# SEU-dynamical-models/Manifold-based-optical-flow-method

Measured on AMD Instinct MI355X. Metric: flow timesteps/sec on 160k-vertex mesh, higher is better.
Workload: dtype f32

## Files before the change

include/mof.h:

```cpp
#ifndef MOF_H_
#define MOF_H_

#include <stdint.h>

#ifdef __cplusplus
extern "C" {
#endif

#define MOF_ABI_VERSION 4

#define MOF_OK 0
#define MOF_E_ARG (-1)
#define MOF_E_HIP (-2)
#define MOF_E_NOCONV (-3)
#define MOF_E_STATE (-4)

#define MOF_GEOM_F32_POINTS 1u
#define MOF_NO_REORDER 2u

#define MOF_PREC_F64 0
#define MOF_PREC_MIXED 1

#define MOF_IO_DEVICE 1u
#define MOF_NO_BLOCK_JACOBI 2u
// ... 114 lines not shown

int mof_csv_write(const char *path, const double *data, int64_t rows, int64_t cols,
                  int32_t threads);
int mof_csv_shape(const char *path, int64_t *rows, int64_t *cols);
#define MOF_CSV_ROUND_TRIP 1u
int mof_csv_read(const char *path, double *out, int64_t rows, int64_t cols, uint32_t flags,
                 int32_t threads);

int mof_ply_info(const char *path, int64_t *n_vertices, int64_t *n_faces, uint32_t *has_normals);
int mof_ply_read(const char *path, float *points, int64_t *triangles, float *normals);
int mof_point_normals(const float *points, const int64_t *triangles, int64_t N, int64_t M,
                      float *normals);
int mof_cell_areas(const float *points, const int64_t *triangles, int64_t N, int64_t M,
                   double *areas);

int mof_amg_probe(const int32_t *tri, const double *e, int32_t N, int32_t M, int32_t *n_levels,
                  int32_t *level_nodes, double *qtq_err, double *max_curl);

int mof_index_probe(const int32_t *tri, int32_t N, int32_t M, uint32_t flags, int32_t sym, int64_t *sell_nb,
                    int32_t *sell_off, int32_t *col, int32_t *mir, uint32_t *packed, int32_t *sym_used,
                    int32_t *packed_used);
int mof_test_force_index32(int32_t on);

int mof_xcd_map_check(int32_t nblk, int32_t batch, int32_t group);
int mof_xcd_batch_cap(int64_t nblk, int32_t group, int32_t *batch);

typedef struct mof_dd mof_dd;

typedef struct mof_dd_info {
    int32_t nparts;
    int32_t local_parts;
    int32_t rank;
    int32_t max_neighbours;
    int32_t max_owned;
    int32_t pad_;
    int64_t ghost_rows;
    int64_t send_rows;
    double ms_setup;
} mof_dd_info;

#define MOF_DD_ID_BYTES 128

int mof_partition_rcb(const double *xyz, int32_t N, int32_t nparts, int32_t *part);

int mof_dd_plan_info(const int32_t *tri, int32_t N, int32_t M, int32_t nparts, const int32_t *part,
                     int32_t *n_own, int32_t *n_ghost, int32_t *n_nbr, int32_t *n_tri,
// ... 37 lines not shown
```

manifold-based-optical-flow-method_amd/csrc/mof_abi.cpp:

```cpp
#include <algorithm>
#include <chrono>
#include <cmath>
#include <cstring>
#include <cstdio>
#include <cstdlib>
#include <functional>
#include <future>
#include <memory>
#include <mutex>
#include <new>

#include "mof_amg.h"
#include "mof_dd.h"
#include "mof_hostio.h"
#include "mof_internal.h"

namespace {

thread_local std::string g_err;

template <class F>
int guarded(F &&f) {
    try {
        f();
// ... 324 lines not shown
                release_f64();
                break;
            }
            used_f64 = true;
        } else {
            ensure(prec);
        }
        st.iterations += solve(rp, only.data());
        for (int32_t b = 0; b < nb; ++b)
            if (only[b] && !failed(b) && prec == MOF_PREC_F64) st.recovered_f64++;
    }
    if (used_f64) release_f64();
    for (int32_t b = 0; b < nb; ++b)
        if (first[b] && !failed(b)) st.recovered++;
}

}

int mof_io_guard(const std::function<void()> &f) { return guarded(f); }

namespace mof {

std::atomic<int> g_force_index32{0};

void mesh_set_own(mof_mesh *m, int32_t nown) {
    MOF_HIP(hipSetDevice(m->device));
    m->n_own = nown;
    const int sym = knob(Knob::SymReads) ? (knob_int(Knob::SymReads, 0) != 0) : -1;
    std::shared_ptr<const MirrorTable> mt;
    {
        MeshShared *sh = m->shared.get();
        std::unique_lock<std::mutex> lk;
        if (sh) lk = std::unique_lock<std::mutex>(sh->mu);
        if (sh && sh->mirror && sh->mirror->nown == nown && sh->mirror->sym == sym) {
            mt = sh->mirror;
        } else {
            auto t = std::make_shared<MirrorTable>();
            t->nown = nown;
            t->sym = sym;
            t->table = sell_mirror(m->pat, nown, sym, &t->used);
            if (t->used) t->packed = sell_index_pack(m->pat, t->table);
            if (sh) sh->mirror = t;
            mt = t;
        }
    }
    m->sym_reads = mt->used;
    const std::vector<int32_t> &mir = mt->table;
    m->sell_mir.alloc(mir.size());
    m->sell_mir.upload(mir.data(), mir.size(), m->stream);
    m->idx_packed = !mt->packed.empty() && !g_force_index32.load();
    if (m->idx_packed) {
        m->sell_idx.alloc(mt->packed.size());
        m->sell_idx.upload(mt->packed.data(), mt->packed.size(), m->stream);
    }
    int64_t own = 0;
    for (int32_t v : mir) own += v >= 0 && !(v & kMirT);
    m->blocks_read = own;
    MOF_HIP(hipStreamSynchronize(m->stream));
}

constexpr int32_t kRowsPerWindow = 256;

void mesh_prepare_host(mof_mesh *m, const double *xyz, const double *nrm, const int32_t *tri,
                       const double *area, int32_t N, int32_t M, uint32_t flags, const int32_t *perm_in,
                       const int32_t *tri_ids) {
    m->N = N;
    m->n_own = N;
    m->M = M;
    m->flags = flags;
    double t0 = now_ms();
    MOF_REQUIRE(N > 0 && M > 0, "mesh needs N > 0 vertices and M > 0 triangles");
    for (int64_t q = 0; q < 3 * (int64_t)M; ++q)
        MOF_REQUIRE(tri[q] >= 0 && tri[q] < N, "triangle vertex index out of range");
    m->perm.resize(N);
    m->tperm.resize(M);
    for (int32_t i = 0; i < N; ++i) m->perm[i] = i;
    for (int32_t T = 0; T < M; ++T) m->tperm[T] = T;
// ... 692 lines not shown
        const std::vector<double> zero(3 * (size_t)std::max(N, M), 0.0);
        mof::mesh_prepare_host(&m, zero.data(), zero.data(), tri, zero.data(), N, M, flags, nullptr, nullptr);
        const mof::Pattern &P = m.pat;
        bool used = false;
        const std::vector<int32_t> table = mof::sell_mirror(P, N, sym < 0 ? -1 : (sym != 0), &used);
        const std::vector<uint32_t> pk = used ? mof::sell_index_pack(P, table) : std::vector<uint32_t>();
        *sell_nb = P.sell_nb();
        if (sym_used) *sym_used = used;
        if (packed_used) *packed_used = !pk.empty();
        if (sell_off) std::copy(P.sell_off.begin(), P.sell_off.end(), sell_off);
        if (col) std::copy(P.sell_col.begin(), P.sell_col.end(), col);
        if (mir) std::copy(table.begin(), table.end(), mir);
        if (packed) {
            std::fill(packed, packed + P.sell_nb(), 0u);
            std::copy(pk.begin(), pk.end(), packed);
        }
    });
}

int mof_test_force_index32(int32_t on) {
    return guarded([&] { mof::g_force_index32.store(on != 0); });
}

int mof_xcd_map_check(int32_t nblk, int32_t batch, int32_t group) {
    return guarded([&] {
        MOF_REQUIRE(nblk > 0 && batch > 0 && group >= 0, "bad arguments");
        MOF_REQUIRE(mof::xcd_map_covers(nblk, batch, group), "XCD order does not cover every (row block, system) once");
    });
}

int mof_xcd_batch_cap(int64_t nblk, int32_t group, int32_t *batch) {
    return guarded([&] {
        MOF_REQUIRE(nblk > 0 && group >= 0 && batch, "bad arguments");
        *batch = mof::xcd_batch_cap_host(nblk, group);
    });
}

int mof_bench_spmv(mof_mesh *m, uint32_t precision, int32_t batch, int32_t reps,
                   double *ms_per_launch, double *bytes_per_launch) {
    return guarded([&] {
        MOF_REQUIRE(m && ms_per_launch && bytes_per_launch, "NULL argument");
        MOF_REQUIRE(reps > 0, "reps must be positive");
        mof::mesh_join_prep(m);
        DeviceGuard dg(m->device);
        *ms_per_launch = mof::bench_spmv(m, precision, batch, reps, m->stream, bytes_per_launch);
    });
// ... 4 lines not shown
```

manifold-based-optical-flow-method_amd/csrc/mof_internal.h:

```cpp
#pragma once

#include <hip/hip_runtime.h>

#include <atomic>
#include <cstdint>
#include <cstdlib>
#include <functional>
#include <future>
#include <memory>
#include <mutex>
#include <string>
#include <type_traits>
#include <vector>

#include "../../include/mof.h"
#include "mof_knobs.h"

namespace mof {

constexpr int kWG = 256;
constexpr int kSlice = 64;

struct Error {
    int code;
// ... 54 lines not shown
    std::vector<int32_t> vptr, vcol;
    std::vector<int32_t> cptr, clist;
    int32_t nslices = 0;
    std::vector<int32_t> sell_off;
    std::vector<int32_t> sell_col;
    std::vector<int32_t> sell_blk;
    std::vector<int32_t> blk_row;
    std::vector<int32_t> diag_pos;
    std::vector<int32_t> tsell_off;
    std::vector<int32_t> tinc;
    std::vector<int32_t> tslot;
    int32_t max_w = 0;
    int64_t sell_nb() const { return sell_off.empty() ? 0 : sell_off.back(); }
    int64_t tsell_nb() const { return tsell_off.empty() ? 0 : tsell_off.back(); }
    int32_t nblocks() const { return (int32_t)vcol.size(); }
};

void build_pattern(const int32_t *tri, int32_t N, int32_t M, Pattern &pat,
                   const int32_t *torder = nullptr);
std::vector<int32_t> rcm_order(const Pattern &pat);
std::vector<int32_t> sell_mirror(const Pattern &pat, int32_t nown, int sym, bool *used);
std::vector<uint32_t> sell_index_pack(const Pattern &pat, const std::vector<int32_t> &mir);
extern std::atomic<int> g_force_index32;

struct Workspace {
    int32_t cap = 0;
    int32_t nblk = 0;
    DevArray<double> u64, fc;
    DevArray<float> u32;
    DevArray<float> A32;
    DevArray<double> A64;
    DevArray<double> dinv64;
    DevArray<float> dinv32;
    DevArray<double> rhs;
    DevArray<double> x64, r64;
    DevArray<double> vx, vr, vz, vp, vq;
    DevArray<double> part_pq;
    DevArray<double> part_rzrr;
    DevArray<double> part_rr0;
    DevArray<double> part_dx;
    DevArray<double> sc;
    DevArray<double> sysd;
    DevArray<int32_t> sysi;
    DevArray<int32_t> smap;
    DevArray<double> dt;
    DevArray<double> Ibuf;
    DevArray<double> Iint;
    DevArray<double> Vbuf;
    bool u64_stale = false;
    const double *J0 = nullptr, *J1 = nullptr;
    int32_t JB = 0;
};


enum SysD { SD_TOL2 = 0, SD_RR = 1, SD_FF = 2, SD_REL = 3, SD_RR0 = 4, SD_BEST = 5, SD_OUTER = 6, SD_EST = 7,
            SD_XMAX = 8 };
enum SysI { SI_CONV = 0, SI_ACTIVE = 1, SI_FAILED = 2, SI_ITSUM = 3, SI_BEST_IT = 4, SI_FAIL_IT = 5, SI_FAIL_WHY = 6,
            SI_ITMAX = 7, SI_MET = 8 };
enum FailWhy { FW_BREAKDOWN = 1, FW_DIVERGED = 2, FW_STALLED = 3, FW_MAXITER = 4, FW_RESIDUAL = 5 };
constexpr int kSysStride = 12;

struct AmgDevice;
// ... 26 lines not shown

struct mof_mesh {
    int32_t N = 0, M = 0, device = 0;
    std::mutex prep_mu;
    std::future<void> prep;
    std::exception_ptr prep_err;
    int32_t n_own = 0;
    uint32_t flags = 0;
    hipStream_t stream = nullptr;
    mof::Pattern pat;
    std::vector<int32_t> perm, inv;
    std::vector<int32_t> tperm, tinv;
    std::vector<int32_t> agg_order;
    mof::DevArray<int32_t> perm_d;
    mof::DevArray<int32_t> tri_orig;
    mof::DevArray<int32_t> icol;
    mof::DevArray<int32_t> tri, vptr, vcol, cptr, clist, sell_off, sell_col, sell_blk, blk_row,
        diag_pos, tsell_off, tinc, tslot;
    mof::DevArray<int32_t> sell_mir;
    int64_t blocks_read = 0;
    bool sym_reads = false;
    mof::DevArray<uint32_t> sell_idx;
    bool idx_packed = false;
    mof::DevArray<double> e, gw, iw, area, a2;
    mof::DevArray<double> a2s64, w12_64;
    mof::DevArray<float> a2s32, w12_32;
    double a2s_lambda = 0.0;
    bool a2s_valid = false;
    mof::DevArray<double> Aexp, fexp;
    mof::Workspace ws;
    bool have_last_A = false;
    double ms_geometry = 0.0, ms_pattern = 0.0;
    int32_t *h_sysi = nullptr;
    double *h_sysd = nullptr;
    int32_t h_cap = 0;
    std::vector<hipEvent_t> spmv_events;
    std::vector<int32_t> iter_hint;
    mof::AmgDevice *amg = nullptr;
    mof::HostStage *stage = nullptr;
    mof::DevArray<double> hin[2], hout[2];
    std::shared_ptr<mof::MeshShared> shared;
    hipEvent_t hev[6] = {nullptr, nullptr, nullptr, nullptr, nullptr, nullptr};
    mof::WaveState *wave = nullptr;
    mof::StreamState *sline = nullptr;
};

// ... 105 lines not shown
```

manifold-based-optical-flow-method_amd/csrc/mof_pattern.cpp:

```cpp
#include <algorithm>
#include <chrono>

#include "mof_internal.h"

namespace mof {

void build_pattern(const int32_t *tri, int32_t N, int32_t M, Pattern &pat, const int32_t *torder) {
    MOF_REQUIRE(N > 0 && M > 0, "mesh needs N > 0 vertices and M > 0 triangles");
    MOF_REQUIRE((int64_t)M * 9 < (int64_t)INT32_MAX, "too many triangles for int32 term codes");
    for (int64_t q = 0; q < 3 * (int64_t)M; ++q)
        MOF_REQUIRE(tri[q] >= 0 && tri[q] < N, "triangle vertex index out of range");
    pat.N = N;
    pat.M = M;

    std::vector<int64_t> inc(N + 1, 0);
    for (int64_t q = 0; q < 3 * (int64_t)M; ++q) inc[tri[q] + 1]++;
    for (int32_t i = 0; i < N; ++i) inc[i + 1] += inc[i];
    std::vector<int32_t> cand(3 * inc[N] + N);
    std::vector<int64_t> cfill(N);
    std::vector<int64_t> cbase(N + 1);
    for (int32_t i = 0; i <= N; ++i) cbase[i] = 3 * inc[i] + i;
    for (int32_t i = 0; i < N; ++i) {
        cfill[i] = cbase[i];
        cand[cfill[i]++] = i;
// ... 179 lines not shown
}

std::vector<uint32_t> sell_index_pack(const Pattern &pat, const std::vector<int32_t> &mir) {
    const int64_t snb = pat.sell_off[pat.nslices];
    if (snb >= kIdxMaxNb || (int64_t)mir.size() != snb) return {};
    std::vector<uint32_t> out((size_t)snb, (uint32_t)(uint16_t)kIdxPad << 16);
    for (int32_t s = 0; s < pat.nslices; ++s) {
        const int32_t w = (pat.sell_off[s + 1] - pat.sell_off[s]) / kSlice;
        for (int32_t l = 0; l < kSlice; ++l) {
            const int32_t i = s * kSlice + l;
            if (i >= pat.N) break;
            for (int32_t t = 0; t < w; ++t) {
                const int64_t pos = pat.sell_off[s] + (int64_t)t * kSlice + l;
                if (mir[pos] < 0) continue;
                const int64_t dcol = (int64_t)pat.sell_col[pos] - i;
                const int64_t dpos = (int64_t)(mir[pos] & kMirPos) - pos;
                const bool tr = (mir[pos] & kMirT) != 0;
                if (dcol < -32768 || dcol > 32767 || dpos <= kIdxPad || dpos > 32767 || tr != (dpos != 0)) return {};
                out[pos] = (uint32_t)(uint16_t)(int16_t)dcol | ((uint32_t)(uint16_t)(int16_t)dpos << 16);
            }
        }
    }
    return out;
}

std::vector<int32_t> rcm_order(const Pattern &pat) {
    const int32_t N = pat.N;
    std::vector<int32_t> deg(N), order, perm(N, -1);
    order.reserve(N);
    for (int32_t i = 0; i < N; ++i) deg[i] = pat.vptr[i + 1] - pat.vptr[i];
    std::vector<int32_t> level(N, -1), queue;
    queue.reserve(N);
    auto far = [&](int32_t s) {
        std::vector<int32_t> seen_list{s};
        level[s] = 0;
        size_t h = 0;
        int32_t last = s;
        while (h < seen_list.size()) {
            const int32_t v = seen_list[h++];
            if (level[v] > level[last] || (level[v] == level[last] && deg[v] < deg[last])) last = v;
            for (int32_t q = pat.vptr[v]; q < pat.vptr[v + 1]; ++q) {
                const int32_t w = pat.vcol[q];
                if (level[w] < 0) {
                    level[w] = level[v] + 1;
                    seen_list.push_back(w);
                }
// ... 34 lines not shown
```

manifold-based-optical-flow-method_amd/csrc/mof_pcg.hip:

```cpp
#include <algorithm>
#include <cstdio>
#include <cstdlib>
#include <chrono>
#include <cmath>

#include <hip/hip_ext.h>

#include "mof_dd.h"
#include "mof_internal.h"
#include "mof_rowkern.h"

namespace mof {

thread_local double g_fetch_ms = 0.0;
thread_local int64_t g_fetch_n = 0;

namespace {

template <typename V>
struct OpArgs {
    int32_t N, M;
    const int32_t *sell_off, *sell_col;
    const V *a2s;
    const int32_t *tsell_off;
// ... 114 lines not shown
#pragma unroll
            for (int u = 0; u < U; ++u) {
                const int c = q[u].y;
                const V2 ui = c == 0 ? P0[u] : (c == 1 ? P1[u] : P2[u]);
                const V2 uj = c == 0 ? P1[u] : (c == 1 ? P2[u] : P0[u]);
                const V2 uk = c == 0 ? P2[u] : (c == 1 ? P0[u] : P1[u]);
                const V si = ui.x * xi.x + ui.y * xi.y;
                const V sj = uj.x * xj[u].x + uj.y * xj[u].y;
                const V sk = uk.x * xk[u].x + uk.y * xk[u].y;
                const V cc = (t0 + u < w) ? w12[u] * ((si + si) + sj + sk) : (V)0;
                a0 += ui.x * cc;
                a1 += ui.y * cc;
            }
        }
    }
    y0 = a0;
    y1 = a1;
}

__device__ __forceinline__ double dot3_np(const double *x, const double *y) {
    return fma(x[2], y[2], fma(x[1], y[1], __dmul_rn(x[0], y[0])));
}

template <int NS>
__device__ __forceinline__ void rcn_a2(const OpArgs<double> &op, const int32_t (&bs)[NS], int32_t i,
                                       const double *__restrict__ x64, double (&acc)[NS][2]) {
#pragma clang fp contract(off)
    const int32_t s = i >> 6, l = i & 63;
    const int32_t o = op.sell_off[s];
    const int32_t w = (op.sell_off[s + 1] - o) >> 6;
    for (int32_t t0 = 0; t0 < w; t0 += kResU) {
        int32_t j[kResU];
        double blk[kResU][4];
#pragma unroll
        for (int u = 0; u < kResU; ++u) j[u] = op.sell_col[(int64_t)o + min(t0 + u, w - 1) * kSlice + l];
#pragma unroll
        for (int u = 0; u < kResU; ++u) ld_blk(op.a2s, (int64_t)o + min(t0 + u, w - 1) * kSlice + l, blk[u]);
#pragma unroll
        for (int u = 0; u < kResU; ++u) {
            const bool on = t0 + u < w;
#pragma unroll
            for (int t = 0; t < NS; ++t) {
                const double2 xj = ld2(x64 + 2 * ((int64_t)bs[t] * op.N + j[u]));
                acc[t][0] += on ? blk[u][0] * xj.x + blk[u][1] * xj.y : 0.0;
                acc[t][1] += on ? blk[u][2] * xj.x + blk[u][3] * xj.y : 0.0;
            }
        }
    }
}
template <int NS>
struct RcnRow {
    double2 xi[NS];
    double Ii[NS];
    double ei[6];
};
template <int NS>
__device__ __forceinline__ void rcn_row(const OpArgs<double> &op, const int32_t (&bs)[NS], int32_t i,
                                        const double *__restrict__ x64, RcnRow<NS> &R) {
#pragma unroll
    for (int t = 0; t < NS; ++t) {
        R.xi[t] = ld2(x64 + 2 * ((int64_t)bs[t] * op.N + i));
        R.Ii[t] = op.I0[(int64_t)bs[t] * op.ldI + i];
    }
#pragma unroll
    for (int q = 0; q < 6; ++q) R.ei[q] = op.e[6 * (int64_t)i + q];
}
template <int NS>
__device__ __forceinline__ void rcn_tri(const OpArgs<double> &op, const int32_t (&bs)[NS], int4 q,
                                        const double *__restrict__ x64, const RcnRow<NS> &R,
                                        double (&val)[NS][2]) {
#pragma clang fp contract(off)
    double g[9], ej[6], ek[6], Ij[NS], Ik[NS], wt;
    double2 xj[NS], xk[NS];
    const int64_t T = min(q.x, op.M - 1);
#pragma unroll
    for (int k = 0; k < 9; ++k) g[k] = op.gw[9 * T + k];
#pragma unroll
    for (int k = 0; k < 6; ++k) {
        ej[k] = op.e[6 * (int64_t)q.z + k];
        ek[k] = op.e[6 * (int64_t)q.w + k];
    }
#pragma unroll
    for (int t = 0; t < NS; ++t) {
        const double *Ib = op.I0 + (int64_t)bs[t] * op.ldI;
        const int64_t vb = (int64_t)bs[t] * op.N;
        Ij[t] = Ib[q.z];
        Ik[t] = Ib[q.w];
        xj[t] = ld2(x64 + 2 * (vb + q.z));
        xk[t] = ld2(x64 + 2 * (vb + q.w));
    }
    wt = op.w12[q.x];
    const int c = q.y;
#pragma unroll
    for (int t = 0; t < NS; ++t) {
        const double c0 = c == 0 ? R.Ii[t] : (c == 1 ? Ik[t] : Ij[t]);
        const double c1 = c == 0 ? Ij[t] : (c == 1 ? R.Ii[t] : Ik[t]);
        const double c2 = c == 0 ? Ik[t] : (c == 1 ? Ij[t] : R.Ii[t]);
        double gI[3];
#pragma unroll
        for (int d = 0; d < 3; ++d) gI[d] = (c0 * g[d] + c1 * g[3 + d]) + c2 * g[6 + d];
        const double2 ui = make_double2(dot3_np(gI, R.ei), dot3_np(gI, R.ei + 3));
        const double2 uj = make_double2(dot3_np(gI, ej), dot3_np(gI, ej + 3));
        const double2 uk = make_double2(dot3_np(gI, ek), dot3_np(gI, ek + 3));
        const double si = ui.x * R.xi[t].x + ui.y * R.xi[t].y;
        const double sj = uj.x * xj[t].x + uj.y * xj[t].y;
        const double sk = uk.x * xk[t].x + uk.y * xk[t].y;
        const double cc = wt * ((si + si) + sj + sk);
        val[t][0] = ui.x * cc;
        val[t][1] = ui.y * cc;
    }
}

template <int NS>
__device__ __forceinline__ void apply_row_rcn(const OpArgs<double> &op, const int32_t (&bs)[NS], int32_t i,
                                              const double *__restrict__ x64, double (&y)[NS][2]) {
#pragma clang fp contract(off)
    static_assert(kRcU == 1, "one incidence per load batch");
    const int32_t s = i >> 6, l = i & 63;
    double acc[NS][2];
#pragma unroll
    for (int t = 0; t < NS; ++t) acc[t][0] = acc[t][1] = 0.0;
    rcn_a2<NS>(op, bs, i, x64, acc);
    RcnRow<NS> R;
    rcn_row<NS>(op, bs, i, x64, R);
    const int32_t o = op.tsell_off[s];
    const int32_t w = (op.tsell_off[s + 1] - o) >> 6;
    if (kRcPre && w <= kRcPre) {
        constexpr int P = kRcPre > 0 ? kRcPre : 1;
        int4 qs[P];
#pragma unroll
        for (int t0 = 0; t0 < P; ++t0)
            if (t0 < w) qs[t0] = op.tinc[(int64_t)o + t0 * kSlice + l];
#pragma unroll
// ... 480 lines not shown
            ff += f.x * f.x + f.y * f.y;
        }
    }
    double v[2] = {rr, ff};
    block_sum_q<2, NQ>(v, lds);
    if (tid == 0 && rb < rd.nmax) {
        double *o = part + 2 * red_rec(rd, B, b, rb);
        o[0] = v[0];
        o[1] = v[1];
    }
}
__global__ __launch_bounds__(kWG) void k_residual(OpArgs<double> op, int32_t nblk, int32_t B, RedArgs rd,
                                                  const double *__restrict__ rhs,
                                                  const double *__restrict__ x64,
                                                  const int32_t *__restrict__ sysi,
                                                  double *__restrict__ r64,
                                                  double *__restrict__ part) {
    int32_t rb, b;
    if (!xcd_map(nblk, B, rb, b, kGrpRes)) return;
    residual_rows<1>(op, B, rd, rhs, x64, sysi, r64, part, rb, b);
}

constexpr int kResNS = 2;
template <int NS>
__global__ __launch_bounds__(kWG) void k_residual_rcn(OpArgs<double> op, int32_t nblk, int32_t B, RedArgs rd,
                                                      const double *__restrict__ rhs,
                                                      const double *__restrict__ x64,
                                                      const int32_t *__restrict__ sysi,
                                                      double *__restrict__ r64,
                                                      double *__restrict__ part) {
    __shared__ double lds[8 * NS];
    int32_t rb, bp;
    if (!xcd_map(nblk, (B + NS - 1) / NS, rb, bp, kGrpRes)) return;
    int32_t bs[NS];
    bool act[NS], any = false;
#pragma unroll
    for (int t = 0; t < NS; ++t) {
        bs[t] = min(NS * bp + t, B - 1);
        act[t] = NS * bp + t < B && sysi[bs[t] * kSysStride + SI_ACTIVE] != 0;
        any |= act[t];
    }
    if (!any) return;
    const int32_t N = op.N;
    double v[2 * NS];
#pragma unroll
    for (int t = 0; t < 2 * NS; ++t) v[t] = 0.0;
#pragma unroll
    for (int r = 0; r < kRows; ++r) {
        const int32_t i = rb * kRowsPerWG + r * kWG + threadIdx.x;
        if (i >= N) break;
        double y[NS][2];
        apply_row_rcn<NS>(op, bs, i, x64, y);
#pragma unroll
        for (int t = 0; t < NS; ++t) {
            const int64_t vi = (int64_t)bs[t] * N + i;
            const double2 f = *reinterpret_cast<const double2 *>(rhs + 2 * vi);
            const double r0 = f.x - y[t][0], r1 = f.y - y[t][1];
            if (act[t]) *reinterpret_cast<double2 *>(r64 + 2 * vi) = make_double2(r0, r1);
            if (i < rd.nown) {
                v[2 * t] += r0 * r0 + r1 * r1;
                v[2 * t + 1] += f.x * f.x + f.y * f.y;
            }
        }
    }
    block_sum<2 * NS>(v, lds);
    if (threadIdx.x == 0) {
#pragma unroll
        for (int t = 0; t < NS; ++t) {
            if (!act[t]) continue;
            double *o = part + 2 * red_rec(rd, B, bs[t], rb);
            o[0] = v[2 * t];
            o[1] = v[2 * t + 1];
        }
    }
}

template <int NT = kWG>
__device__ __forceinline__ void reduce_max_sys(const double *part, const RedArgs &rdx, int32_t B, int32_t b,
                                               double (&out)[2], double *lds) {
    out[0] = out[1] = 0.0;
    for (int32_t q = 0; q < rdx.P; ++q) {
        const double *p = part + 2 * ((int64_t)q * B + b) * rdx.nmax;
        for (int32_t w = threadIdx.x; w < rdx.nmax; w += NT) {
            out[0] = fmax(out[0], p[2 * (int64_t)w]);
            out[1] = fmax(out[1], p[2 * (int64_t)w + 1]);
        }
    }
    block_max<2, NT>(out, lds);
}

template <int NT = kWG>
__device__ __forceinline__ void outer_check_sys(const RedArgs &rd, int32_t B, const double *__restrict__ part,
                                                const RedArgs &rdx, const double *__restrict__ part_dx,
                                                int32_t first, double rtol, double etol,
                                                double *__restrict__ sysd, int32_t *__restrict__ sysi,
                                                int32_t b) {
    __shared__ double lds[2 * (NT / 64)];
// ... 88 lines not shown
    op.e = m->e.p;
    op.I0 = m->ws.J0;
    op.ldI = m->N;
    return op;
}

OpArgs<double> op64(mof_mesh *m) {
    return make_op<double>(m, m->a2s64.p, m->w12_64.p, m->ws.u64_stale ? nullptr : m->ws.u64.p);
}

template <typename V>
MatArgs<V> make_mat(mof_mesh *m, const V *A) {
    MatArgs<V> mt;
    mt.sell_nb = m->pat.sell_nb();
    mt.sell_off = m->sell_off.p;
    mt.sell_col = m->sell_col.p;
    mt.sell_mir = m->sym_reads ? m->sell_mir.p : nullptr;
    mt.sell_idx = sizeof(V) == 4 && m->sym_reads && m->idx_packed ? m->sell_idx.p : nullptr;
    mt.vptr = m->sym_reads ? nullptr : m->vptr.p;
    mt.A = A;
    return mt;
}

template <typename... Args>
void launch_residual(mof_mesh *m, int32_t nblk, int32_t B, hipStream_t s, RedArgs rd, Args... args) {
    const OpArgs<double> op = op64(m);
    if (op.u)
        k_residual<<<dim3(xcd_grid(nblk, B, kGrpRes)), kWG, 0, s>>>(op, nblk, B, rd, args...);
    else
        k_residual_rcn<kResNS><<<dim3(xcd_grid(nblk, (B + kResNS - 1) / kResNS, kGrpRes)), kWG, 0, s>>>(
            op, nblk, B, rd, args...);
}

template <typename V>
PcgArgs<V> make_args(mof_mesh *m, int32_t B, const MatArgs<V> &mat, const V *dinv) {
    Workspace &w = m->ws;
    PcgArgs<V> a;
    a.N = m->N;
    a.nblk = w.nblk;
    a.B = B;
    a.sm = sys_all(B);
    a.selfred = 0;
    a.mat = mat;
    a.dinv = dinv;
    a.x = reinterpret_cast<V *>(w.vx.p);
    a.r = reinterpret_cast<V *>(w.vr.p);
    a.z = reinterpret_cast<V *>(w.vz.p);
    a.p = reinterpret_cast<V *>(w.vp.p);
    a.q = reinterpret_cast<V *>(w.vq.p);
    a.part_pq = w.part_pq.p;
    a.part_rzrr = w.part_rzrr.p;
    a.sysd = w.sysd.p;
    a.sysi = w.sysi.p;
    a.red = RedArgs{1, 0, w.nblk, m->N};
// ... 341 lines not shown
        MOF_HIP(hipStreamSynchronize(m->stream));
        return;
    }
    w.cap = B;
    w.nblk = (int32_t)((N + kRowsPerWG - 1) / kRowsPerWG);
    w.u64.release();
    w.u32.release();
    w.fc.release();
    w.dinv64.alloc(4 * N * B);
    w.dinv32.alloc(4 * N * B);
    w.rhs.alloc(2 * N * B);
    w.x64.alloc(2 * N * B);
    w.r64.alloc(2 * N * B);
    w.vx.alloc(2 * N * B);
    w.vr.alloc(2 * N * B);
    w.vz.alloc(2 * N * B);
    w.vp.alloc(2 * N * B);
    w.vq.alloc(2 * N * B);
    w.part_pq.alloc(2 * (size_t)w.nblk * B);
    w.part_rzrr.alloc((size_t)4 * w.nblk * B);
    w.sc.alloc((size_t)6 * B);
    w.sc.zero(m->stream);
    w.part_rr0.alloc((size_t)2 * w.nblk * B);
    w.part_dx.alloc((size_t)2 * ((N + kWG - 1) / kWG) * B);
    w.sysd.alloc((size_t)kSysStride * B);
    w.sysi.alloc((size_t)kSysStride * B);
    w.smap.alloc((size_t)B);
    w.dt.alloc(B);
    w.Ibuf.alloc(2 * N * B);
    w.Iint.alloc(2 * N * B);
    w.Vbuf.alloc(2 * N * B);
    if (m->h_cap < B) {
        if (m->h_sysi) (void)hipHostFree(m->h_sysi);
        if (m->h_sysd) (void)hipHostFree(m->h_sysd);
        m->h_sysi = nullptr;
        m->h_sysd = nullptr;
        MOF_HIP(hipHostMalloc((void **)&m->h_sysi, sizeof(int32_t) * kSysStride * B, 0));
        MOF_HIP(hipHostMalloc((void **)&m->h_sysd, sizeof(double) * kSysStride * B, 0));
        m->h_cap = B;
    }
    MOF_HIP(hipStreamSynchronize(m->stream));
}

constexpr int32_t kFusedMaxBlk = 16;
bool fused_eligible(const mof_mesh *m, const SolveParams &sp, const uint8_t *only) {
    if (sp.fused == 0 || only || sp.precision != MOF_PREC_F64 || sp.amg || sp.fail_at_max_iter) return false;
// ... 417 lines not shown
```

manifold-based-optical-flow-method_amd/mofhip/_lib.py:

```python
from __future__ import annotations

import ctypes
import os
import subprocess
import threading

import numpy as np

PKG_DIR = os.path.dirname(os.path.abspath(__file__))
ROOT_DIR = os.path.dirname(PKG_DIR)
CSRC_DIR = os.path.join(ROOT_DIR, "csrc")
LIB_PATH = os.environ.get("MOFHIP_LIB") or os.path.join(PKG_DIR, "libmofhip.so")

MOF_ABI_VERSION = 4

MOF_OK = 0
MOF_E_ARG = -1
MOF_E_HIP = -2
MOF_E_NOCONV = -3
MOF_E_STATE = -4

MOF_GEOM_F32_POINTS = 1
MOF_NO_REORDER = 2
MOF_PREC_F64 = 0
# ... 3 lines not shown
MOF_TIME_SPMV = 4
MOF_PRECOND_AMG = 8
MOF_NO_RECOVERY = 16
MOF_SOLVE_FUSED = 128
MOF_SOLVE_EAGER = 256
MOF_CSV_ROUND_TRIP = 1
MOF_COORDS_F32 = 32
MOF_DD_STAGED = 64
MOF_WAVE_PHASE = 512
MOF_CSR_A2 = 0
MOF_CSR_A_LAST = 1

EXPORTS = (
    "mof_version", "mof_abi_version", "mof_last_error", "mof_device_count", "mof_mesh_create", "mof_mesh_clone",
    "mof_mesh_destroy", "mof_mesh_get_info", "mof_geometry_export", "mof_csr_export",
    "mof_assemble", "mof_solve_range", "mof_bench_spmv", "mof_velocity_vectors",
    "mof_csv_write", "mof_csv_shape", "mof_csv_read", "mof_ply_info", "mof_ply_read",
    "mof_point_normals", "mof_cell_areas", "mof_singularities", "mof_amg_probe",
    "mof_partition_rcb", "mof_dd_plan_info", "mof_dd_create", "mof_dd_unique_id",
    "mof_dd_create_rank", "mof_dd_destroy", "mof_dd_get_info", "mof_dd_solve_range",
    "mof_dd_test_fail_recovery_alloc", "mof_mesh_prepare", "mof_mesh_sync",
    "mof_singularities_compact", "mof_xcd_map_check", "mof_xcd_batch_cap", "mof_dd_create_rank_host",
    "mof_index_probe", "mof_test_force_index32", "mof_wave_speed", "mof_streamline_map", "mof_streamlines",
    "mof_test_streamline_pass",
)


class MofError(RuntimeError):

    def __init__(self, code, msg):
        super().__init__("libmofhip error %d: %s" % (code, msg))
        self.code = code


class NotConverged(MofError):
    pass


class MofOpts(ctypes.Structure):
    _fields_ = [
        ("struct_size", ctypes.c_uint32), ("precision", ctypes.c_uint32),
        ("flags", ctypes.c_uint32), ("batch", ctypes.c_int32), ("max_iter", ctypes.c_int32),
        ("max_outer", ctypes.c_int32), ("rtol", ctypes.c_double),
        ("inner_rtol", ctypes.c_double), ("stream", ctypes.c_void_p),
        ("etol", ctypes.c_double),
    ]

# ... 83 lines not shown
            "mof_mesh_get_info": ([P, P], ctypes.c_int),
            "mof_geometry_export": ([P, P, P, P], ctypes.c_int),
            "mof_csr_export": ([P, i32, i32, P, P, P, P], ctypes.c_int),
            "mof_assemble": ([P, P, P, f64, f64, P], ctypes.c_int),
            "mof_solve_range": ([P, P, P, P, i32, i32, i32, f64, P, P, P], ctypes.c_int),
            "mof_bench_spmv": ([P, u32, i32, i32, P, P], ctypes.c_int),
            "mof_velocity_vectors": ([i32, P, P, i32, i32, P, P, u32, P], ctypes.c_int),
            "mof_csv_write": ([ctypes.c_char_p, P, i64, i64, i32], ctypes.c_int),
            "mof_csv_shape": ([ctypes.c_char_p, P, P], ctypes.c_int),
            "mof_csv_read": ([ctypes.c_char_p, P, i64, i64, u32, i32], ctypes.c_int),
            "mof_ply_info": ([ctypes.c_char_p, P, P, P], ctypes.c_int),
            "mof_ply_read": ([ctypes.c_char_p, P, P, P], ctypes.c_int),
            "mof_point_normals": ([P, P, i64, i64, P], ctypes.c_int),
            "mof_cell_areas": ([P, P, i64, i64, P], ctypes.c_int),
            "mof_wave_speed": ([P, P, i32, f64, u32, i32, P, P, P, P, P], ctypes.c_int),
            "mof_streamline_map": ([P, P, i32, u32, P, P, P], ctypes.c_int),
            "mof_streamlines": ([P, P, i32, i32, u32, P, i64, i64, P, P, P, P], ctypes.c_int),
            "mof_test_streamline_pass": ([i32], ctypes.c_int),
            "mof_singularities": ([i32, P, P, i32, i32, P, i32, f64, u32, P, P, P, P, P],
                                  ctypes.c_int),
            "mof_amg_probe": ([P, P, i32, i32, P, P, P, P], ctypes.c_int),
            "mof_index_probe": ([P, i32, i32, u32, i32, P, P, P, P, P, P, P], ctypes.c_int),
            "mof_test_force_index32": ([i32], ctypes.c_int),
            "mof_xcd_map_check": ([i32, i32, i32], ctypes.c_int),
            "mof_xcd_batch_cap": ([i64, i32, P], ctypes.c_int),
            "mof_singularities_compact": ([i32, P, P, i32, i32, P, i32, f64, u32, P, i64, P, P, P, P, P,
                                           P, P], ctypes.c_int),
            "mof_partition_rcb": ([P, i32, i32, P], ctypes.c_int),
            "mof_dd_plan_info": ([P, i32, i32, i32, P, P, P, P, P, P], ctypes.c_int),
            "mof_dd_create": ([P, P, P, P, i32, i32, i32, P, i32, u32, P], ctypes.c_int),
            "mof_dd_unique_id": ([P], ctypes.c_int),
            "mof_dd_create_rank": ([P, P, P, P, i32, i32, i32, P, i32, P, i32, u32, P],
                                   ctypes.c_int),
            "mof_dd_create_rank_host": ([P, P, P, P, i32, i32, i32, P, i32, P, i32, u32, P],
                                        ctypes.c_int),
            "mof_dd_destroy": ([P], ctypes.c_int),
            "mof_dd_get_info": ([P, P], ctypes.c_int),
            "mof_mesh_prepare": ([P, P], ctypes.c_int),
            "mof_mesh_sync": ([P], ctypes.c_int),
            "mof_dd_test_fail_recovery_alloc": ([P, i32], ctypes.c_int),
            "mof_dd_solve_range": ([P, P, P, P, i32, i32, i32, f64, P, P, P], ctypes.c_int),
        }
        for name, (args, res) in sig.items():
            if os.environ.get("MOFHIP_LIB") and not hasattr(L, name):
                continue
            fn = getattr(L, name)
# ... 33 lines not shown
```

manifold-based-optical-flow-method_amd/mofhip/mesh.py:

```python
from __future__ import annotations

import ctypes
import threading
import time

import numpy as np

from . import _lib as L


def _f64(a):
    return np.ascontiguousarray(a, dtype=np.float64)


class DeviceMesh:

    def __init__(self, coordinates, normals, triangles, areas, device: int = 0,
                 reorder: bool = True):
        coords = np.asarray(coordinates)
        tri = np.asarray(triangles)
        if coords.ndim != 2 or coords.shape[1] != 3:
            raise ValueError("coordinates must be (N, 3)")
        if tri.ndim != 2 or tri.shape[1] != 3:
            raise ValueError("triangles must be (M, 3)")
# ... 234 lines not shown
    flags = 0 if reorder else L.MOF_NO_REORDER
    nb, su, pu = ctypes.c_int64(0), ctypes.c_int32(0), ctypes.c_int32(0)
    L.check(L.lib().mof_index_probe(L.ptr(T), N, M, flags, int(sym), ctypes.byref(nb), None, None, None, None,
                                    None, None))
    off = np.zeros((N + 63) // 64 + 1, dtype=np.int32)
    col = np.zeros(nb.value, dtype=np.int32)
    mir = np.zeros(nb.value, dtype=np.int32)
    packed = np.zeros(nb.value, dtype=np.uint32)
    L.check(L.lib().mof_index_probe(L.ptr(T), N, M, flags, int(sym), ctypes.byref(nb), L.ptr(off), L.ptr(col),
                                    L.ptr(mir), L.ptr(packed), ctypes.byref(su), ctypes.byref(pu)))
    return {"sell_off": off, "col": col, "mir": mir, "packed": packed, "sym_used": bool(su.value),
            "packed_used": bool(pu.value)}


class force_index32:

    def __enter__(self):
        L.check(L.lib().mof_test_force_index32(1))
        return self

    def __exit__(self, *exc):
        L.check(L.lib().mof_test_force_index32(0))
        return False
```

Before: 4033.

## Stage per-slice operator data in LDS for batched residual kernel

Adds a residual kernel that loads one 64-row slice's A2 blocks, column indices, edge frames and triangle incidence/gradient data into shared memory once. Several waves then reuse that staged data across multiple system pairs, and a small fold kernel reduces the per-slice partial norms into the existing reduction records. The aim is to cut repeated global reads of matrix and geometry data across systems in the batch. The cost is a large dynamic LDS allocation per block (up to 160 KB), which limits occupancy, plus an extra launch and workspace buffer. The older per-row kernel remains as a fallback when a slice does not fit.

```diff
diff --git a/include/mof.h b/include/mof.h
--- a/include/mof.h
+++ b/include/mof.h
@@ -160,6 +160,12 @@
                     int32_t *packed_used);
 int mof_test_force_index32(int32_t on);
 
+int mof_residual_probe(const int32_t *tri, int32_t N, int32_t M, uint32_t flags, int64_t *staged_bytes,
+                       int32_t *staged_used);
+int mof_test_force_residual_rows(int32_t on);
+int mof_test_force_residual_trips(int32_t on);
+int mof_test_residual_launches(int64_t *counts);
+
 int mof_xcd_map_check(int32_t nblk, int32_t batch, int32_t group);
 int mof_xcd_batch_cap(int64_t nblk, int32_t group, int32_t *batch);
 
diff --git a/manifold-based-optical-flow-method_amd/csrc/mof_abi.cpp b/manifold-based-optical-flow-method_amd/csrc/mof_abi.cpp
--- a/manifold-based-optical-flow-method_amd/csrc/mof_abi.cpp
+++ b/manifold-based-optical-flow-method_amd/csrc/mof_abi.cpp
@@ -370,6 +370,9 @@
 namespace mof {
 
 std::atomic<int> g_force_index32{0};
+std::atomic<int> g_force_residual_rows{0};
+std::atomic<int> g_force_residual_trips{0};
+std::atomic<int64_t> g_residual_launches[3];
 
 void mesh_set_own(mof_mesh *m, int32_t nown) {
     MOF_HIP(hipSetDevice(m->device));
@@ -401,6 +404,8 @@
         m->sell_idx.alloc(mt->packed.size());
         m->sell_idx.upload(mt->packed.data(), mt->packed.size(), m->stream);
     }
+    m->res_lds_bytes = res_staged_bytes(m->pat);
+    m->res_lds = m->res_lds_bytes <= kResLdsCap && !g_force_residual_rows.load();
     int64_t own = 0;
     for (int32_t v : mir) own += v >= 0 && !(v & kMirT);
     m->blocks_read = own;
@@ -1139,6 +1144,33 @@
     return guarded([&] { mof::g_force_index32.store(on != 0); });
 }
 
+int mof_residual_probe(const int32_t *tri, int32_t N, int32_t M, uint32_t flags, int64_t *staged_bytes,
+                       int32_t *staged_used) {
+    return guarded([&] {
+        MOF_REQUIRE(tri && staged_bytes && N > 0 && M > 0, "bad arguments");
+        mof_mesh m;
+        const std::vector<double> zero(3 * (size_t)std::max(N, M), 0.0);
+        mof::mesh_prepare_host(&m, zero.data(), zero.data(), tri, zero.data(), N, M, flags, nullptr, nullptr);
+        *staged_bytes = mof::res_staged_bytes(m.pat);
+        if (staged_used) *staged_used = *staged_bytes <= mof::kResLdsCap;
+    });
+}
+
+int mof_test_force_residual_rows(int32_t on) {
+    return guarded([&] { mof::g_force_residual_rows.store(on != 0); });
+}
+
+int mof_test_force_residual_trips(int32_t on) {
+    return guarded([&] { mof::g_force_residual_trips.store(on != 0); });
+}
+
+int mof_test_residual_launches(int64_t *counts) {
+    return guarded([&] {
+        MOF_REQUIRE(counts, "NULL argument");
+        for (int k = 0; k < 3; ++k) counts[k] = mof::g_residual_launches[k].load();
+    });
+}
+
 int mof_xcd_map_check(int32_t nblk, int32_t batch, int32_t group) {
     return guarded([&] {
         MOF_REQUIRE(nblk > 0 && batch > 0 && group >= 0, "bad arguments");
diff --git a/manifold-based-optical-flow-method_amd/csrc/mof_internal.h b/manifold-based-optical-flow-method_amd/csrc/mof_internal.h
--- a/manifold-based-optical-flow-method_amd/csrc/mof_internal.h
+++ b/manifold-based-optical-flow-method_amd/csrc/mof_internal.h
@@ -100,6 +100,14 @@
 std::vector<int32_t> sell_mirror(const Pattern &pat, int32_t nown, int sym, bool *used);
 std::vector<uint32_t> sell_index_pack(const Pattern &pat, const std::vector<int32_t> &mir);
 extern std::atomic<int> g_force_index32;
+constexpr int64_t kResLdsCap = 160 * 1024;
+inline int64_t res_slice_bytes(int32_t w_a2, int32_t w_inc) {
+    return (int64_t)kSlice * ((int64_t)w_a2 * 36 + (int64_t)w_inc * 192 + 48);
+}
+int64_t res_staged_bytes(const Pattern &pat);
+extern std::atomic<int> g_force_residual_rows;
+extern std::atomic<int> g_force_residual_trips;
+extern std::atomic<int64_t> g_residual_launches[3];
 
 struct Workspace {
     int32_t cap = 0;
@@ -116,6 +124,7 @@
     DevArray<double> part_pq;
     DevArray<double> part_rzrr;
     DevArray<double> part_rr0;
+    DevArray<double> res_spart;
     DevArray<double> part_dx;
     DevArray<double> sc;
     DevArray<double> sysd;
@@ -188,6 +197,8 @@
     bool sym_reads = false;
     mof::DevArray<uint32_t> sell_idx;
     bool idx_packed = false;
+    int64_t res_lds_bytes = 0;
+    bool res_lds = false;
     mof::DevArray<double> e, gw, iw, area, a2;
     mof::DevArray<double> a2s64, w12_64;
     mof::DevArray<float> a2s32, w12_32;
diff --git a/manifold-based-optical-flow-method_amd/csrc/mof_pattern.cpp b/manifold-based-optical-flow-method_amd/csrc/mof_pattern.cpp
--- a/manifold-based-optical-flow-method_amd/csrc/mof_pattern.cpp
+++ b/manifold-based-optical-flow-method_amd/csrc/mof_pattern.cpp
@@ -225,6 +225,14 @@
         }
     }
     return out;
+}
+
+int64_t res_staged_bytes(const Pattern &pat) {
+    int64_t mx = 0;
+    for (int32_t s = 0; s < pat.nslices; ++s)
+        mx = std::max(mx, res_slice_bytes((pat.sell_off[s + 1] - pat.sell_off[s]) / kSlice,
+                                          (pat.tsell_off[s + 1] - pat.tsell_off[s]) / kSlice));
+    return mx;
 }
 
 std::vector<int32_t> rcm_order(const Pattern &pat) {
diff --git a/manifold-based-optical-flow-method_amd/csrc/mof_pcg.hip b/manifold-based-optical-flow-method_amd/csrc/mof_pcg.hip
--- a/manifold-based-optical-flow-method_amd/csrc/mof_pcg.hip
+++ b/manifold-based-optical-flow-method_amd/csrc/mof_pcg.hip
@@ -160,6 +160,11 @@
     return fma(x[2], y[2], fma(x[1], y[1], __dmul_rn(x[0], y[0])));
 }
 
+__device__ __forceinline__ void rcn_a2_term(const double (&blk)[4], double2 xj, bool on, double (&acc)[2]) {
+#pragma clang fp contract(off)
+    acc[0] += on ? blk[0] * xj.x + blk[1] * xj.y : 0.0;
+    acc[1] += on ? blk[2] * xj.x + blk[3] * xj.y : 0.0;
+}
 template <int NS>
 __device__ __forceinline__ void rcn_a2(const OpArgs<double> &op, const int32_t (&bs)[NS], int32_t i,
                                        const double *__restrict__ x64, double (&acc)[NS][2]) {
@@ -178,11 +183,8 @@
         for (int u = 0; u < kResU; ++u) {
             const bool on = t0 + u < w;
 #pragma unroll
-            for (int t = 0; t < NS; ++t) {
-                const double2 xj = ld2(x64 + 2 * ((int64_t)bs[t] * op.N + j[u]));
-                acc[t][0] += on ? blk[u][0] * xj.x + blk[u][1] * xj.y : 0.0;
-                acc[t][1] += on ? blk[u][2] * xj.x + blk[u][3] * xj.y : 0.0;
-            }
+            for (int t = 0; t < NS; ++t)
+                rcn_a2_term(blk[u], ld2(x64 + 2 * ((int64_t)bs[t] * op.N + j[u])), on, acc[t]);
         }
     }
 }
@@ -203,6 +205,27 @@
 #pragma unroll
     for (int q = 0; q < 6; ++q) R.ei[q] = op.e[6 * (int64_t)i + q];
 }
+__device__ __forceinline__ void rcn_tri_term(int c, const double (&g)[9], const double (&ei)[6],
+                                             const double (&ej)[6], const double (&ek)[6], double wt, double Ii,
+                                             double Ij, double Ik, double2 xi, double2 xj, double2 xk,
+                                             double (&val)[2]) {
+#pragma clang fp contract(off)
+    const double c0 = c == 0 ? Ii : (c == 1 ? Ik : Ij);
+    const double c1 = c == 0 ? Ij : (c == 1 ? Ii : Ik);
+    const double c2 = c == 0 ? Ik : (c == 1 ? Ij : Ii);
+    double gI[3];
+#pragma unroll
+    for (int d = 0; d < 3; ++d) gI[d] = (c0 * g[d] + c1 * g[3 + d]) + c2 * g[6 + d];
+    const double2 ui = make_double2(dot3_np(gI, ei), dot3_np(gI, ei + 3));
+    const double2 uj = make_double2(dot3_np(gI, ej), dot3_np(gI, ej + 3));
+    const double2 uk = make_double2(dot3_np(gI, ek), dot3_np(gI, ek + 3));
+    const double si = ui.x * xi.x + ui.y * xi.y;
+    const double sj = uj.x * xj.x + uj.y * xj.y;
+    const double sk = uk.x * xk.x + uk.y * xk.y;
+    const double cc = wt * ((si + si) + sj + sk);
+    val[0] = ui.x * cc;
+    val[1] = ui.y * cc;
+}
 template <int NS>
 __device__ __forceinline__ void rcn_tri(const OpArgs<double> &op, const int32_t (&bs)[NS], int4 q,
                                         const double *__restrict__ x64, const RcnRow<NS> &R,
@@ -228,25 +251,8 @@
         xk[t] = ld2(x64 + 2 * (vb + q.w));
     }
     wt = op.w12[q.x];
-    const int c = q.y;
-#pragma unroll
-    for (int t = 0; t < NS; ++t) {
-        const double c0 = c == 0 ? R.Ii[t] : (c == 1 ? Ik[t] : Ij[t]);
-        const double c1 = c == 0 ? Ij[t] : (c == 1 ? R.Ii[t] : Ik[t]);
-        const double c2 = c == 0 ? Ik[t] : (c == 1 ? Ij[t] : R.Ii[t]);
-        double gI[3];
-#pragma unroll
-        for (int d = 0; d < 3; ++d) gI[d] = (c0 * g[d] + c1 * g[3 + d]) + c2 * g[6 + d];
-        const double2 ui = make_double2(dot3_np(gI, R.ei), dot3_np(gI, R.ei + 3));
-        const double2 uj = make_double2(dot3_np(gI, ej), dot3_np(gI, ej + 3));
-        const double2 uk = make_double2(dot3_np(gI, ek), dot3_np(gI, ek + 3));
-        const double si = ui.x * R.xi[t].x + ui.y * R.xi[t].y;
-        const double sj = uj.x * xj[t].x + uj.y * xj[t].y;
-        const double sk = uk.x * xk[t].x + uk.y * xk[t].y;
-        const double cc = wt * ((si + si) + sj + sk);
-        val[t][0] = ui.x * cc;
-        val[t][1] = ui.y * cc;
-    }
+#pragma unroll
+    for (int t = 0; t < NS; ++t) rcn_tri_term(q.y, g, R.ei, ej, ek, wt, R.Ii[t], Ij[t], Ik[t], R.xi[t], xj[t], xk[t], val[t]);
 }
 
 template <int NS>
@@ -773,6 +779,17 @@
 }
 
 constexpr int kResNS = 2;
+__device__ __forceinline__ void rcn_out(int64_t vi, bool own, bool act, const double (&y)[2],
+                                        const double *__restrict__ rhs, double *__restrict__ r64, double &rr,
+                                        double &ff) {
+    const double2 f = *reinterpret_cast<const double2 *>(rhs + 2 * vi);
+    const double r0 = f.x - y[0], r1 = f.y - y[1];
+    if (act) *reinterpret_cast<double2 *>(r64 + 2 * vi) = make_double2(r0, r1);
+    if (own) {
+        rr += r0 * r0 + r1 * r1;
+        ff += f.x * f.x + f.y * f.y;
+    }
+}
 template <int NS>
 __global__ __launch_bounds__(kWG) void k_residual_rcn(OpArgs<double> op, int32_t nblk, int32_t B, RedArgs rd,
                                                       const double *__restrict__ rhs,
@@ -804,14 +821,7 @@
         apply_row_rcn<NS>(op, bs, i, x64, y);
 #pragma unroll
         for (int t = 0; t < NS; ++t) {
-            const int64_t vi = (int64_t)bs[t] * N + i;
-            const double2 f = *reinterpret_cast<const double2 *>(rhs + 2 * vi);
-            const double r0 = f.x - y[t][0], r1 = f.y - y[t][1];
-            if (act[t]) *reinterpret_cast<double2 *>(r64 + 2 * vi) = make_double2(r0, r1);
-            if (i < rd.nown) {
-                v[2 * t] += r0 * r0 + r1 * r1;
-                v[2 * t + 1] += f.x * f.x + f.y * f.y;
-            }
+            rcn_out((int64_t)bs[t] * N + i, i < rd.nown, act[t], y[t], rhs, r64, v[2 * t], v[2 * t + 1]);
         }
     }
     block_sum<2 * NS>(v, lds);
@@ -824,6 +834,183 @@
             o[1] = v[2 * t + 1];
         }
     }
+}
+
+constexpr int kLdsW = 16, kLdsTrips = 4;
+constexpr int kLdsUA = 4;
+constexpr int32_t kGrpResLds = 1;
+constexpr int64_t kLdsFill = 1024;
+template <int NS, int W, int TRIPS>
+__global__ __launch_bounds__(64 * W) void k_residual_lds(OpArgs<double> op, int32_t nsl, int32_t B, RedArgs rd,
+                                                         const double *__restrict__ rhs,
+                                                         const double *__restrict__ x64,
+                                                         const int32_t *__restrict__ sysi,
+                                                         double *__restrict__ r64,
+                                                         double *__restrict__ spart) {
+    extern __shared__ double2 sm[];
+    constexpr int NT = 64 * W, PW = W * TRIPS;
+    const int32_t npair = (B + NS - 1) / NS;
+    int32_t s, chunk;
+    if (!xcd_map(nsl, (npair + PW - 1) / PW, s, chunk, kGrpResLds)) return;
+    const int32_t wv = threadIdx.x >> 6, l = threadIdx.x & 63;
+    {
+        bool any = false;
+        for (int32_t q = l; q < PW * NS; q += 64) {
+            const int32_t b = chunk * PW * NS + q;
+            any |= b < B && sysi[min(b, B - 1) * kSysStride + SI_ACTIVE] != 0;
+        }
+        if (__ballot(any) == 0) return;
+    }
+    const int32_t N = op.N;
+    const int32_t o = op.sell_off[s], wa = (op.sell_off[s + 1] - o) >> 6;
+    const int32_t to = op.tsell_off[s], wt = (op.tsell_off[s + 1] - to) >> 6;
+    double2 *const E = sm, *const BLK = sm + 3 * 64, *const INC = BLK + 2 * 64 * wa;
+    int32_t *const COL = reinterpret_cast<int32_t *>(INC + 12 * 64 * wt);
+    for (int32_t q = threadIdx.x; q < wa * 64; q += NT) {
+        const int32_t t = q >> 6, ll = q & 63;
+        COL[q] = op.sell_col[(int64_t)o + q];
+        const double2 *bp = reinterpret_cast<const double2 *>(op.a2s) + 2 * ((int64_t)o + q);
+        BLK[(2 * t) * 64 + ll] = bp[0];
+        BLK[(2 * t + 1) * 64 + ll] = bp[1];
+    }
+    for (int32_t q = threadIdx.x; q < 3 * 64; q += NT) {
+        const int32_t k = q >> 6, ll = q & 63;
+        E[q] = ld2(op.e + 6 * (int64_t)min(64 * s + ll, N - 1) + 2 * k);
+    }
+    for (int32_t q = threadIdx.x; q < wt * 4 * 64; q += NT) {
+        const int32_t ll = q & 63, part = (q >> 6) & 3, t = q >> 8;
+        const int4 e = op.tinc[(int64_t)to + t * 64 + ll];
+        double2 *P = INC + (12 * t) * 64 + ll;
+        if (part == 0) {
+            const double *g = op.gw + 9 * (int64_t)min(e.x, op.M - 1);
+            *reinterpret_cast<int4 *>(P) = e;
+            P[1 * 64] = make_double2(g[0], g[1]);
+            P[2 * 64] = make_double2(g[2], g[3]);
+            P[3 * 64] = make_double2(g[4], g[5]);
+        } else if (part == 1) {
+            const double *g = op.gw + 9 * (int64_t)min(e.x, op.M - 1);
+            P[4 * 64] = make_double2(g[6], g[7]);
+            P[5 * 64] = make_double2(g[8], op.w12[e.x]);
+        } else {
+            const double *ev = op.e + 6 * (int64_t)(part == 2 ? e.z : e.w);
+            double2 *Q = P + (part == 2 ? 6 : 9) * 64;
+            Q[0] = ld2(ev);
+            Q[64] = ld2(ev + 2);
+            Q[128] = ld2(ev + 4);
+        }
+    }
+    __syncthreads();
+    const int32_t i = 64 * s + l;
+#pragma unroll 1
+    for (int trip = 0; trip < TRIPS; ++trip) {
+        const int32_t bp = chunk * PW + trip * W + wv;
+        if (bp >= npair) break;
+        int32_t bs[NS];
+        bool act[NS], any = false;
+#pragma unroll
+        for (int t = 0; t < NS; ++t) {
+            bs[t] = min(NS * bp + t, B - 1);
+            act[t] = NS * bp + t < B && sysi[bs[t] * kSysStride + SI_ACTIVE] != 0;
+            any |= act[t];
+        }
+        if (!any) continue;
+        double v[2 * NS];
+#pragma unroll
+        for (int t = 0; t < 2 * NS; ++t) v[t] = 0.0;
+        if (i < N) {
+            double acc[NS][2];
+#pragma unroll
+            for (int t = 0; t < NS; ++t) acc[t][0] = acc[t][1] = 0.0;
+            for (int32_t t0 = 0; t0 < wa; t0 += kLdsUA) {
+                double2 xj[kLdsUA][NS];
+#pragma unroll
+                for (int u = 0; u < kLdsUA; ++u) {
+                    const int32_t j = COL[min(t0 + u, wa - 1) * 64 + l];
+#pragma unroll
+                    for (int t = 0; t < NS; ++t) xj[u][t] = ld2(x64 + 2 * ((int64_t)bs[t] * N + j));
+                }
+#pragma unroll
+                for (int u = 0; u < kLdsUA; ++u) {
+                    const int32_t tt = min(t0 + u, wa - 1);
+                    const double2 b0 = BLK[(2 * tt) * 64 + l], b1 = BLK[(2 * tt + 1) * 64 + l];
+                    const double blk[4] = {b0.x, b0.y, b1.x, b1.y};
+#pragma unroll
+                    for (int t = 0; t < NS; ++t) rcn_a2_term(blk, xj[u][t], t0 + u < wa, acc[t]);
+                }
+            }
+            double2 xi[NS];
+            double Ii[NS];
+#pragma unroll
+            for (int t = 0; t < NS; ++t) {
+                xi[t] = ld2(x64 + 2 * ((int64_t)bs[t] * N + i));
+                Ii[t] = op.I0[(int64_t)bs[t] * op.ldI + i];
+            }
+            const double2 e0 = E[l], e1 = E[64 + l], e2 = E[128 + l];
+            const double ei[6] = {e0.x, e0.y, e1.x, e1.y, e2.x, e2.y};
+            for (int32_t t0 = 0; t0 < wt; ++t0) {
+                const double2 *P = INC + (12 * t0) * 64 + l;
+                const int4 q = *reinterpret_cast<const int4 *>(P);
+                double Ij[NS], Ik[NS];
+                double2 xj[NS], xk[NS];
+#pragma unroll
+                for (int t = 0; t < NS; ++t) {
+                    const double *Ib = op.I0 + (int64_t)bs[t] * op.ldI;
+                    const int64_t vb = (int64_t)bs[t] * N;
+                    Ij[t] = Ib[q.z];
+                    Ik[t] = Ib[q.w];
+                    xj[t] = ld2(x64 + 2 * (vb + q.z));
+                    xk[t] = ld2(x64 + 2 * (vb + q.w));
+                }
+                const double2 g01 = P[64], g23 = P[2 * 64], g45 = P[3 * 64], g67 = P[4 * 64], g8w = P[5 * 64];
+                const double2 j0 = P[6 * 64], j1 = P[7 * 64], j2 = P[8 * 64];
+                const double2 k0 = P[9 * 64], k1 = P[10 * 64], k2 = P[11 * 64];
+                const double g[9] = {g01.x, g01.y, g23.x, g23.y, g45.x, g45.y, g67.x, g67.y, g8w.x};
+                const double ej[6] = {j0.x, j0.y, j1.x, j1.y, j2.x, j2.y};
+                const double ek[6] = {k0.x, k0.y, k1.x, k1.y, k2.x, k2.y};
+#pragma unroll
+                for (int t = 0; t < NS; ++t) {
+                    double val[2];
+                    rcn_tri_term(q.y, g, ei, ej, ek, g8w.y, Ii[t], Ij[t], Ik[t], xi[t], xj[t], xk[t], val);
+                    acc[t][0] += val[0];
+                    acc[t][1] += val[1];
+                }
+            }
+#pragma unroll
+            for (int t = 0; t < NS; ++t)
+                rcn_out((int64_t)bs[t] * N + i, i < rd.nown, act[t], acc[t], rhs, r64, v[2 * t], v[2 * t + 1]);
+        }
+#pragma unroll
+        for (int t = 0; t < 2 * NS; ++t) v[t] = wave_sum(v[t]);
+        if (l == 0) {
+#pragma unroll
+            for (int t = 0; t < NS; ++t) {
+                if (!act[t]) continue;
+                double *op_ = spart + 2 * ((int64_t)bs[t] * nsl + s);
+                op_[0] = v[2 * t];
+                op_[1] = v[2 * t + 1];
+            }
+        }
+    }
+}
+__global__ __launch_bounds__(kWG) void k_residual_fold(int32_t nsl, int32_t nblk, int32_t B, RedArgs rd,
+                                                       const int32_t *__restrict__ sysi,
+                                                       const double *__restrict__ spart,
+                                                       double *__restrict__ part) {
+    const int64_t q = (int64_t)blockIdx.x * kWG + threadIdx.x;
+    if (q >= (int64_t)B * nblk) return;
+    const int32_t b = (int32_t)(q / nblk), rb = (int32_t)(q - (int64_t)b * nblk);
+    if (!sysi[b * kSysStride + SI_ACTIVE]) return;
+    double w[4][2];
+#pragma unroll
+    for (int k = 0; k < 4; ++k) {
+        const int32_t s = 4 * rb + k;
+        const double *p = spart + 2 * ((int64_t)b * nsl + min(s, nsl - 1));
+        w[k][0] = s < nsl ? p[0] : 0.0;
+        w[k][1] = s < nsl ? p[1] : 0.0;
+    }
+    double *out = part + 2 * red_rec(rd, B, b, rb);
+    out[0] = ((w[0][0] + w[1][0]) + w[2][0]) + w[3][0];
+    out[1] = ((w[0][1] + w[1][1]) + w[2][1]) + w[3][1];
 }
 
 template <int NT = kWG>
@@ -958,14 +1145,44 @@
     return mt;
 }
 
+void launch_residual_lds(mof_mesh *m, const OpArgs<double> &op, int32_t nblk, int32_t B, hipStream_t s, RedArgs rd,
+                         const double *rhs, const double *x64, const int32_t *sysi, double *r64, double *part) {
+    constexpr int kMaxDev = 64;
+    static std::once_flag once[kMaxDev];
+    const auto kern = &k_residual_lds<kResNS, kLdsW, kLdsTrips>, kern1 = &k_residual_lds<kResNS, kLdsW, 1>;
+    MOF_REQUIRE(m->device >= 0 && m->device < kMaxDev, "device index out of range");
+    std::call_once(once[m->device], [&] {
+        for (const void *k : {reinterpret_cast<const void *>(kern), reinterpret_cast<const void *>(kern1)})
+            MOF_HIP(hipFuncSetAttribute(k, hipFuncAttributeMaxDynamicSharedMemorySize, (int)kResLdsCap));
+    });
+    const int32_t nsl = m->pat.nslices, npair = (B + kResNS - 1) / kResNS;
+    int32_t nchunk = (npair + kLdsW * kLdsTrips - 1) / (kLdsW * kLdsTrips);
+    const bool one = (int64_t)nsl * nchunk < kLdsFill && !g_force_residual_trips.load();
+    if (one) nchunk = (npair + kLdsW - 1) / kLdsW;
+    MOF_REQUIRE(m->res_lds_bytes <= kResLdsCap && m->ws.res_spart.n >= (size_t)2 * nsl * B,
+                "staged residual: workspace not set up");
+    const unsigned grid = xcd_grid(nsl, nchunk, kGrpResLds);
+    MOF_REQUIRE((int64_t)grid * 64 * kLdsW < ((int64_t)1 << 32), "launch grid past 2^32 work-items");
+    g_residual_launches[one ? 1 : 2]++;
+    (one ? kern1 : kern)<<<dim3(grid), 64 * kLdsW, (size_t)m->res_lds_bytes, s>>>(op, nsl, B, rd, rhs, x64, sysi, r64,
+                                                                                   m->ws.res_spart.p);
+    const int64_t nrec = (int64_t)B * nblk;
+    k_residual_fold<<<dim3((unsigned)((nrec + kWG - 1) / kWG)), kWG, 0, s>>>(nsl, nblk, B, rd, sysi,
+                                                                             m->ws.res_spart.p, part);
+}
+
 template <typename... Args>
 void launch_residual(mof_mesh *m, int32_t nblk, int32_t B, hipStream_t s, RedArgs rd, Args... args) {
     const OpArgs<double> op = op64(m);
     if (op.u)
         k_residual<<<dim3(xcd_grid(nblk, B, kGrpRes)), kWG, 0, s>>>(op, nblk, B, rd, args...);
-    else
+    else if (m->res_lds)
+        launch_residual_lds(m, op, nblk, B, s, rd, args...);
+    else {
+        g_residual_launches[0]++;
         k_residual_rcn<kResNS><<<dim3(xcd_grid(nblk, (B + kResNS - 1) / kResNS, kGrpRes)), kWG, 0, s>>>(
             op, nblk, B, rd, args...);
+    }
 }
 
 template <typename V>
@@ -1353,6 +1570,7 @@
     w.sc.alloc((size_t)6 * B);
     w.sc.zero(m->stream);
     w.part_rr0.alloc((size_t)2 * w.nblk * B);
+    if (m->res_lds) w.res_spart.alloc((size_t)2 * m->pat.nslices * B);
     w.part_dx.alloc((size_t)2 * ((N + kWG - 1) / kWG) * B);
     w.sysd.alloc((size_t)kSysStride * B);
     w.sysi.alloc((size_t)kSysStride * B);
diff --git a/manifold-based-optical-flow-method_amd/mofhip/_lib.py b/manifold-based-optical-flow-method_amd/mofhip/_lib.py
--- a/manifold-based-optical-flow-method_amd/mofhip/_lib.py
+++ b/manifold-based-optical-flow-method_amd/mofhip/_lib.py
@@ -49,7 +49,8 @@
     "mof_dd_test_fail_recovery_alloc", "mof_mesh_prepare", "mof_mesh_sync",
     "mof_singularities_compact", "mof_xcd_map_check", "mof_xcd_batch_cap", "mof_dd_create_rank_host",
     "mof_index_probe", "mof_test_force_index32", "mof_wave_speed", "mof_streamline_map", "mof_streamlines",
-    "mof_test_streamline_pass",
+    "mof_test_streamline_pass", "mof_residual_probe", "mof_test_force_residual_rows",
+    "mof_test_force_residual_trips", "mof_test_residual_launches",
 )
 
 
@@ -179,6 +180,10 @@
             "mof_amg_probe": ([P, P, i32, i32, P, P, P, P], ctypes.c_int),
             "mof_index_probe": ([P, i32, i32, u32, i32, P, P, P, P, P, P, P], ctypes.c_int),
             "mof_test_force_index32": ([i32], ctypes.c_int),
+            "mof_residual_probe": ([P, i32, i32, u32, P, P], ctypes.c_int),
+            "mof_test_force_residual_rows": ([i32], ctypes.c_int),
+            "mof_test_force_residual_trips": ([i32], ctypes.c_int),
+            "mof_test_residual_launches": ([P], ctypes.c_int),
             "mof_xcd_map_check": ([i32, i32, i32], ctypes.c_int),
             "mof_xcd_batch_cap": ([i64, i32, P], ctypes.c_int),
             "mof_singularities_compact": ([i32, P, P, i32, i32, P, i32, f64, u32, P, i64, P, P, P, P, P,
diff --git a/manifold-based-optical-flow-method_amd/mofhip/mesh.py b/manifold-based-optical-flow-method_amd/mofhip/mesh.py
--- a/manifold-based-optical-flow-method_amd/mofhip/mesh.py
+++ b/manifold-based-optical-flow-method_amd/mofhip/mesh.py
@@ -280,3 +280,40 @@
     def __exit__(self, *exc):
         L.check(L.lib().mof_test_force_index32(0))
         return False
+
+
+def residual_probe(triangles, n_vertices: int, reorder: bool = True) -> dict:
+    T = np.ascontiguousarray(triangles, dtype=np.int32)
+    flags = 0 if reorder else L.MOF_NO_REORDER
+    nb, used = ctypes.c_int64(0), ctypes.c_int32(0)
+    L.check(L.lib().mof_residual_probe(L.ptr(T), int(n_vertices), len(T), flags, ctypes.byref(nb),
+                                       ctypes.byref(used)))
+    return {"staged_bytes": int(nb.value), "staged_used": bool(used.value)}
+
+
+class force_residual_rows:
+
+    def __enter__(self):
+        L.check(L.lib().mof_test_force_residual_rows(1))
+        return self
+
+    def __exit__(self, *exc):
+        L.check(L.lib().mof_test_force_residual_rows(0))
+        return False
+
+
+class force_residual_trips:
+
+    def __enter__(self):
+        L.check(L.lib().mof_test_force_residual_trips(1))
+        return self
+
+    def __exit__(self, *exc):
+        L.check(L.lib().mof_test_force_residual_trips(0))
+        return False
+
+
+def residual_launches() -> dict:
+    c = np.zeros(3, dtype=np.int64)
+    L.check(L.lib().mof_test_residual_launches(L.ptr(c)))
+    return {"rows": int(c[0]), "staged_one": int(c[1]), "staged_multi": int(c[2])}
```

Result: faster. 4163 (median of 6 runs) (+3.2%).
